# ubc-vision/quadraturefields

Measured on AMD Instinct MI355X. Metric: rays/sec at 800x800 Lego (mesh-quadrature render: ray/mesh intersection + hash-grid/MLP field + compositing), higher is better.
Workload: dtype f32; 1 GPU; Lego 800x800 (configs[1]), 1xMI355X per frame, fp32 hash-grid + tiny-MLP HIP kernels; rays_per_frame=640000, max_hits=25, triangles=983040, log2_hashmap_size=19, up_sample=1, bvh_fallback_frames=0, overflow_repaired_frames=8, reorigin_rule_redone_frames=0, camera_mismatch_frames=0, frames_in_flight=1

## Files before the change

quadraturefields_amd/build.py:

```python
import os
import subprocess
import sys
from concurrent.futures import ThreadPoolExecutor

PKG_DIR = os.path.dirname(os.path.abspath(__file__))
ROOT = os.path.dirname(PKG_DIR)
CSRC = os.path.join(PKG_DIR, "csrc")
OBJ_DIR = os.path.join(CSRC, "_obj")
LIB_PATH = os.path.join(PKG_DIR, "libqf_hip.so")
ARCH = "gfx950"

SOURCES = [
    ("field_eval.hip", []),
    ("field_eval_bf16.hip", []),
    ("grid_extract.hip", []),
    ("grid_backward.hip", []),
    ("mlp_train.hip", []),
    ("field_train.hip", []),
    ("scan.hip", []),
    ("composite.hip", []),
    ("distortion.hip", []),
    ("optim.hip", []),
    ("frame_metrics.hip", []),
    ("bvh_traverse.hip", ["-ffp-contract=off"]),
    ("raster.hip", ["-ffp-contract=off"]),
    ("sample_pack.hip", ["-ffp-contract=off"]),
    ("texture.hip", ["-ffp-contract=off"]),
    ("bake.hip", ["-ffp-contract=off"]),
    ("grid_march.hip", ["-ffp-contract=off"]),
    ("volumetric.hip", ["-ffp-contract=off"]),
    ("texel_fill.hip", ["-ffp-contract=off"]),
    ("marching_cubes.hip", ["-ffp-contract=off"]),
    ("vertex_clustering.hip", ["-ffp-contract=off"]),
    ("uv_atlas.hip", ["-ffp-contract=off"]),
    ("bvh_build_device.hip", ["-ffp-contract=off"]),
    ("bvh_build.cpp", ["-x", "hip"]),
    ("misc.cpp", ["-x", "hip"]),
    ("frame.cpp", ["-x", "hip"]),
]
COMMON = os.environ.get("QF_EXTRA_HIPCC_FLAGS", "").split() + ["-O3", "-std=c++17", "-fPIC", f"--offload-arch={ARCH}", "-I" + os.path.join(ROOT, "include"),
          "-I" + CSRC, "-Wall", "-Wno-unused-function"]


def _hipcc() -> str:
    for cand in (os.environ.get("HIPCC"), "/opt/rocm/bin/hipcc", "hipcc"):
        if cand and (os.path.isabs(cand) and os.path.exists(cand) or not os.path.isabs(cand)):
            return cand
    raise RuntimeError("hipcc not found")


def _deps(src: str):
    deps = [os.path.join(CSRC, src), os.path.join(ROOT, "include", "qf_hip.h"), os.path.abspath(__file__)]
    deps += [os.path.join(CSRC, f) for f in os.listdir(CSRC) if f.endswith(".h")]
    return deps


def _stale(target: str, deps) -> bool:
    if not os.path.exists(target):
        return True
    t = os.path.getmtime(target)
    return any(os.path.getmtime(d) > t for d in deps)


def _obj(src: str) -> str:
    return os.path.join(OBJ_DIR, os.path.splitext(src)[0] + ".o")


def _compile(item):
    src, extra = item
    obj = _obj(src)
    if not _stale(obj, _deps(src)):
        return obj, False
    cmd = [_hipcc()] + COMMON + extra + ["-c", os.path.join(CSRC, src), "-o", obj]
    proc = subprocess.run(cmd, capture_output=True, text=True)
    if proc.returncode != 0:
        raise RuntimeError("hipcc failed for %s:\n%s\n%s" % (src, " ".join(cmd), proc.stderr))
    if proc.stderr.strip():
        sys.stderr.write(proc.stderr)
    return obj, True


def build(force: bool = False, verbose: bool = False) -> str:
    os.makedirs(OBJ_DIR, exist_ok=True)
    keep = set() if force else {_obj(src) for src, _ in SOURCES}
    for f in os.listdir(OBJ_DIR):
        if os.path.join(OBJ_DIR, f) not in keep:
            os.remove(os.path.join(OBJ_DIR, f))
    with ThreadPoolExecutor(max_workers=4) as pool:
        results = list(pool.map(_compile, SOURCES))
    objs = [o for o, _ in results]
    if any(changed for _, changed in results) or _stale(LIB_PATH, objs):
        cmd = [_hipcc(), "-shared", "-fPIC", f"--offload-arch={ARCH}", "-o", LIB_PATH] + objs
        proc = subprocess.run(cmd, capture_output=True, text=True)
        if proc.returncode != 0:
            raise RuntimeError("link failed:\n%s\n%s" % (" ".join(cmd), proc.stderr))
        if verbose:
            print("linked", LIB_PATH)
    return LIB_PATH


if __name__ == "__main__":
    print(build(force="--force" in sys.argv, verbose=True))
```

quadraturefields_amd/csrc/raster.hip:

```cpp
#include <type_traits>

#include "exact_common.h"

#pragma clang fp contract(off)

namespace {

struct RasterCam {
    float r00, r01, r02, r10, r11, r12, r20, r21, r22;
    float cx, cy, cz;
    float fx, fy, px0, py0;
    int w, h;
};

constexpr float kRasterGuard = 0.25f;

struct SlabArgs {
    float t_lo, t_hi;
    int stop_at;
    uint64_t *keys;
    const float4 *ray_rec;
};

struct TriSetup {
    int x0, x1, y0, y1;
    bool use_edges;
    float ea[3], eb[3], ec[3];
};

__device__ __forceinline__ bool tri_setup(const float4 a, const float4 b, const float4 c, const RasterCam &cam, TriSetup &s)
{
    float minx = INFINITY, maxx = -INFINITY, miny = INFINITY, maxy = -INFINITY;
    int behind = 0;
    const float4 vs[3] = {a, b, c};
    float sxs[3], sys[3];
#pragma unroll
    for (int k = 0; k < 3; ++k) {
        const float dx = vs[k].x - cam.cx, dy = vs[k].y - cam.cy, dz = vs[k].z - cam.cz;
        const float xc = cam.r00 * dx + cam.r10 * dy + cam.r20 * dz;
        const float yc = cam.r01 * dx + cam.r11 * dy + cam.r21 * dz;
        const float zc = cam.r02 * dx + cam.r12 * dy + cam.r22 * dz;
        const float zv = -zc;
        if (!(zv > 1e-6f)) { ++behind; sxs[k] = sys[k] = 0.0f; continue; }
        const float sx = cam.fx * (xc / zv) + cam.px0;
        const float sy = -cam.fy * (yc / zv) + cam.py0;
        sxs[k] = sx; sys[k] = sy;
        minx = fminf(minx, sx); maxx = fmaxf(maxx, sx);
        miny = fminf(miny, sy); maxy = fmaxf(maxy, sy);
    }
    if (behind == 3) return false;
    s.use_edges = false;
    if (behind > 0) {
        s.x0 = 0; s.y0 = 0; s.x1 = cam.w - 1; s.y1 = cam.h - 1;
    } else {
        s.x0 = (int)fmaxf(floorf(minx - kRasterGuard), 0.0f);
        s.y0 = (int)fmaxf(floorf(miny - kRasterGuard), 0.0f);
        s.x1 = (int)fminf(ceilf(maxx + kRasterGuard), (float)(cam.w - 1));
        s.y1 = (int)fminf(ceilf(maxy + kRasterGuard), (float)(cam.h - 1));
        if (!(maxx + kRasterGuard >= 0.0f) || !(maxy + kRasterGuard >= 0.0f) ||
            !(minx - kRasterGuard <= (float)(cam.w - 1)) || !(miny - kRasterGuard <= (float)(cam.h - 1)))
            return false;
        const float area2 = (sxs[1] - sxs[0]) * (sys[2] - sys[0]) - (sys[1] - sys[0]) * (sxs[2] - sxs[0]);
        if (fabsf(area2) > 1e-2f) {
            s.use_edges = true;
            const float sgn = area2 > 0.0f ? 1.0f : -1.0f;
#pragma unroll
            for (int k = 0; k < 3; ++k) {
                const int k1 = (k + 1) % 3;
                const float ex = sxs[k1] - sxs[k], ey = sys[k1] - sys[k];
                s.ea[k] = -sgn * ey;
                s.eb[k] = sgn * ex;
                s.ec[k] = -(s.ea[k] * sxs[k] + s.eb[k] * sys[k]) + (kRasterGuard + 0.05f) * (fabsf(ex) + fabsf(ey)) + 1e-3f;
            }
        }
    }
    return true;
}

constexpr int kBinStage = 256;
constexpr int kBinIdBits = 26;
struct BinStage { int n; int tile[kBinStage]; uint2 rec[kBinStage]; };
struct TileBins {
    int32_t *cursor;
    uint2 *bins;
    int cap;
    BinStage *stage;
};

__device__ __forceinline__ void bin_records(const TileBins &tb, int tile, uint2 rec)
{
    const int lane = (int)__lane_id();
    for (;;) {
        const int t0 = __builtin_amdgcn_readfirstlane(tile);
        const unsigned long long m = __ballot(tile == t0);
        if (tile == t0) {
            const int rank = __popcll(m & ((1ull << lane) - 1ull));
            int base = 0;
            if (rank == 0) base = atomicAdd(&tb.cursor[t0], __popcll(m));
            base = __shfl(base, __ffsll((long long)m) - 1, 64);
            if (base + rank < tb.cap) tb.bins[(int64_t)t0 * tb.cap + base + rank] = rec;
            break;
        }
    }
}

template <int kRasterLanes, bool kWide, bool kSlab = false, bool kBins = false>
__device__ __forceinline__ void raster_triangle(const float4 *__restrict__ tris, int64_t tri_i, int sub, const RasterCam &cam,
                                                const float *__restrict__ rays_o, const float *__restrict__ rays_d,
                                                int max_hits, int32_t *__restrict__ hit_tri, float *__restrict__ hit_t,
                                                int32_t *__restrict__ hit_count, int32_t *__restrict__ overflow,
                                                const bool cam_origin, const SlabArgs slab = SlabArgs(),
                                                const TileBins bins = TileBins())
{
    const float4 a = tris[tri_i * 3 + 0], b = tris[tri_i * 3 + 1], c = tris[tri_i * 3 + 2];
    const int id = __float_as_int(a.w);
    TriSetup ts;
    if (!tri_setup(a, b, c, cam, ts)) return;
    const int x0 = ts.x0, x1 = ts.x1, y0 = ts.y0, y1 = ts.y1;
    const bool use_edges = ts.use_edges;
    const float *ea = ts.ea, *eb = ts.eb, *ec = ts.ec;
    const int bw = x1 - x0 + 1;
    const int total = bw * (y1 - y0 + 1);
    int px = x0 + sub % bw, py = y0 + sub / bw;
    for (int q = sub; q < total; q += kRasterLanes) {
        const int cx_ = px, cy_ = py;
        px += kRasterLanes;
        while (px > x1) { px -= bw; ++py; }
        if (use_edges) {
            const float fx_ = (float)cx_, fy_ = (float)cy_;
            if (ea[0] * fx_ + eb[0] * fy_ + ec[0] < 0.0f || ea[1] * fx_ + eb[1] * fy_ + ec[1] < 0.0f ||
                ea[2] * fx_ + eb[2] * fy_ + ec[2] < 0.0f)
                continue;
        }
        const int64_t ray = (int64_t)cy_ * cam.w + cx_;
        float dx, dy, dz;
        if (kSlab && slab.ray_rec) {
            const float4 rr = slab.ray_rec[ray];
            if (__float_as_int(rr.w) >= slab.stop_at) continue;
            dx = rr.x; dy = rr.y; dz = rr.z;
        } else {
            dx = rays_d[ray * 3]; dy = rays_d[ray * 3 + 1]; dz = rays_d[ray * 3 + 2];
        }
        float ox = cam.cx, oy = cam.cy, oz = cam.cz;
        if (!cam_origin) { ox = rays_o[ray * 3]; oy = rays_o[ray * 3 + 1]; oz = rays_o[ray * 3 + 2]; }
        asm volatile("" : "+v"(ox), "+v"(oy), "+v"(oz), "+v"(dx), "+v"(dy), "+v"(dz));
        float t;
        if (!mt_hit(a, b, c, ox, oy, oz, dx, dy, dz, &t)) continue;
        if (kSlab) {
            if (!(t >= slab.t_lo && t < slab.t_hi)) continue;
            const int slot = atomicAdd(&hit_count[ray], 1);
            if (slot < max_hits) slab.keys[(int64_t)slot * ((int64_t)cam.w * cam.h) + ray] = hit_key(t, id);
            else atomicAdd(overflow, 1);
            continue;
        }
        if (kBins) {
            const int tile = (cy_ >> 3) * ((cam.w + 7) >> 3) + (cx_ >> 3);
            const uint2 rec = make_uint2(__float_as_uint(t), ((uint32_t)id << 6) | (uint32_t)((cy_ & 7) * 8 + (cx_ & 7)));
            const int at = atomicAdd(&bins.stage->n, 1);
            if (at < kBinStage) { bins.stage->tile[at] = tile; bins.stage->rec[at] = rec; }
            else bin_records(bins, tile, rec);
            continue;
        }
        const int slot = atomicAdd(&hit_count[ray], 1);
        if (slot < max_hits) {
            const int64_t at = kWide ? (int64_t)slot * ((int64_t)cam.w * cam.h) + ray : ray * max_hits + slot;
            hit_t[at] = t;
            if (hit_tri) hit_tri[at] = id;
        } else {
            atomicAdd(overflow, 1);
        }
    }
}

template <int kRasterLanes, bool kWide>
__global__ __launch_bounds__(256) void raster_kernel(const float4 *__restrict__ tris, int64_t n_tri, RasterCam cam,
                                                     const float *__restrict__ rays_o, const float *__restrict__ rays_d,
                                                     int max_hits, int32_t *__restrict__ hit_tri, float *__restrict__ hit_t,
                                                     int32_t *__restrict__ hit_count, int32_t *__restrict__ overflow,
                                                     const int32_t *__restrict__ ray_flag)
{
    const int64_t gid = (int64_t)blockIdx.x * blockDim.x + threadIdx.x;
    const int64_t tri_i = gid / kRasterLanes;
    const int sub = (int)(gid % kRasterLanes);
    if (tri_i >= n_tri) return;
    if (ray_flag && *ray_flag) return;
    const bool cam_origin = ray_flag != nullptr;
    raster_triangle<kRasterLanes, kWide>(tris, tri_i, sub, cam, rays_o, rays_d, max_hits, hit_tri, hit_t, hit_count, overflow,
                                         cam_origin);
}

template <int kRasterLanes>
__global__ __launch_bounds__(256) void raster_bins_kernel(const float4 *__restrict__ tris, int64_t n_tri, RasterCam cam,
                                                          const float *__restrict__ rays_o, const float *__restrict__ rays_d,
                                                          int max_hits, int32_t *__restrict__ tile_cursor,
                                                          uint2 *__restrict__ bin_records_out,
                                                          const int32_t *__restrict__ ray_flag)
{
    __shared__ BinStage s_stage[4];
    const int64_t gid = (int64_t)blockIdx.x * blockDim.x + threadIdx.x;
    const int64_t tri_i = gid / kRasterLanes;
    const int sub = (int)(gid % kRasterLanes);
    if (ray_flag && *ray_flag) return;
    const bool cam_origin = ray_flag != nullptr;
    const int lane = (int)(threadIdx.x & 63);
    TileBins tb;
    tb.cursor = tile_cursor;
    tb.bins = bin_records_out;
    tb.cap = 64 * max_hits;
    tb.stage = &s_stage[threadIdx.x >> 6];
    if (lane == 0) tb.stage->n = 0;
    __builtin_amdgcn_fence(__ATOMIC_ACQ_REL, "workgroup");
    __builtin_amdgcn_wave_barrier();
    if (tri_i < n_tri)
        raster_triangle<kRasterLanes, false, false, true>(tris, tri_i, sub, cam, rays_o, rays_d, max_hits, nullptr, nullptr,
                                                          nullptr, nullptr, cam_origin, SlabArgs(), tb);
    __builtin_amdgcn_fence(__ATOMIC_ACQ_REL, "workgroup");
    __builtin_amdgcn_wave_barrier();
    const int n = tb.stage->n < kBinStage ? tb.stage->n : kBinStage;
    for (int i = lane; i < n; i += 64) bin_records(tb, tb.stage->tile[i], tb.stage->rec[i]);
}

__global__ __launch_bounds__(64) void tile_count_kernel(const int32_t *__restrict__ tile_cursor, const uint2 *__restrict__ bins,
                                                        int max_hits, int w, int h, int tiles_x,
                                                        int32_t *__restrict__ hit_count, int32_t *__restrict__ overflow,
                                                        uint64_t *__restrict__ tile_mask)
{
    __shared__ int s_cnt[64];
    const int tile = blockIdx.x, lane = threadIdx.x;
    const int cap = 64 * max_hits;
    const int cursor = tile_cursor[tile];
    const int n = cursor < cap ? cursor : cap;
    const int px = (tile % tiles_x) * 8 + (lane & 7), py = (tile / tiles_x) * 8 + (lane >> 3);
    const bool inside = px < w && py < h;
    int c = 0;
    if (n > 0) {
        s_cnt[lane] = 0;
        __syncthreads();
        const uint2 *run = bins + (int64_t)tile * cap;
        for (int i = lane; i < n; i += 64) atomicAdd(&s_cnt[run[i].y & 63u], 1);
        __syncthreads();
        c = s_cnt[lane];
    }
    int over = c > max_hits ? c - max_hits : 0;
    if (cursor > cap) {
        c = c > max_hits ? c : max_hits + 1;
        over = lane == 0 ? cursor - cap : 0;
    }
    if (inside) hit_count[(int64_t)py * w + px] = c;
    const unsigned long long mask = __ballot(inside && c > max_hits);
    if (mask) {
#pragma unroll
        for (int off = 32; off > 0; off >>= 1) over += __shfl_xor(over, off, 64);
        if (lane == 0) atomicAdd(overflow, over);
    }
    if (lane == 0) tile_mask[tile] = mask;
}

constexpr float kRayPixelTol = 0.02f;
constexpr float kRayUnitTol = 1e-4f;

__device__ __forceinline__ void camera_rays_check(const uint32_t *__restrict__ o_bits, const float *__restrict__ rays_d,
                                                  int64_t n_rays, const RasterCam &cam, int32_t *__restrict__ flag,
                                                  int64_t first, int64_t stride)
{
    const uint32_t c0 = __float_as_uint(cam.cx), c1 = __float_as_uint(cam.cy), c2 = __float_as_uint(cam.cz);
    bool bad = false;
    for (int64_t r = first; r < n_rays; r += stride) {
        const uint32_t o0 = o_bits[r * 3], o1 = o_bits[r * 3 + 1], o2 = o_bits[r * 3 + 2];
        const float dx = rays_d[r * 3], dy = rays_d[r * 3 + 1], dz = rays_d[r * 3 + 2];
        bad = bad || o0 != c0 || o1 != c1 || o2 != c2;
        const float xc = cam.r00 * dx + cam.r10 * dy + cam.r20 * dz;
        const float yc = cam.r01 * dx + cam.r11 * dy + cam.r21 * dz;
        const float zv = -(cam.r02 * dx + cam.r12 * dy + cam.r22 * dz);
        const float sx = cam.fx * (xc / zv) + cam.px0, sy = -cam.fy * (yc / zv) + cam.py0;
        const float px = (float)(int)(r % cam.w), py = (float)(int)(r / cam.w);
        bad = bad || !(zv > 0.0f) || !(fabsf(sx - px) <= kRayPixelTol) || !(fabsf(sy - py) <= kRayPixelTol) ||
              !(fabsf(dx * dx + dy * dy + dz * dz - 1.0f) <= kRayUnitTol);
    }
    if (bad) *flag = 1;
}

__global__ void camera_rays_check_kernel(const uint32_t *__restrict__ o_bits, const float *__restrict__ rays_d, int64_t n_rays,
                                         RasterCam cam, int32_t *__restrict__ flag)
{
    camera_rays_check(o_bits, rays_d, n_rays, cam, flag, (int64_t)blockIdx.x * blockDim.x + threadIdx.x,
                      (int64_t)gridDim.x * blockDim.x);
}

constexpr int kCullChunk = 64;

__global__ __launch_bounds__(256) void chunk_boxes_kernel(const float4 *__restrict__ tris, int64_t n_tri, int n_chunks,
                                                          float4 *__restrict__ boxes)
{
    const int chunk = (int)(((int64_t)blockIdx.x * blockDim.x + threadIdx.x) >> 6), lane = threadIdx.x & 63;
    if (chunk >= n_chunks) return;
    const int64_t t = (int64_t)chunk * kCullChunk + lane;
    float lo[3] = {INFINITY, INFINITY, INFINITY}, hi[3] = {-INFINITY, -INFINITY, -INFINITY};
    if (t < n_tri) {
#pragma unroll
        for (int k = 0; k < 3; ++k) {
            const float4 v = tris[t * 3 + k];
            lo[0] = fminf(lo[0], v.x); lo[1] = fminf(lo[1], v.y); lo[2] = fminf(lo[2], v.z);
            hi[0] = fmaxf(hi[0], v.x); hi[1] = fmaxf(hi[1], v.y); hi[2] = fmaxf(hi[2], v.z);
        }
    }
#pragma unroll
    for (int off = 32; off > 0; off >>= 1) {
#pragma unroll
        for (int k = 0; k < 3; ++k) {
            lo[k] = fminf(lo[k], __shfl_xor(lo[k], off, 64));
            hi[k] = fmaxf(hi[k], __shfl_xor(hi[k], off, 64));
        }
    }
    if (lane == 0) {
        boxes[chunk * 2 + 0] = make_float4(lo[0], lo[1], lo[2], 0.0f);
        boxes[chunk * 2 + 1] = make_float4(hi[0], hi[1], hi[2], 0.0f);
    }
}

__global__ void cull_chunks_kernel(const float4 *__restrict__ boxes, int n_chunks, RasterCam cam, int32_t *__restrict__ visible,
                                   int32_t *__restrict__ counters, int parity, const uint32_t *__restrict__ o_bits,
                                   const float *__restrict__ rays_d, int64_t n_rays, int32_t *__restrict__ ray_flag)
{
    const int chunk = blockIdx.x * blockDim.x + threadIdx.x;
    if (chunk == 0) counters[parity ^ 1] = 0;
    if (ray_flag) camera_rays_check(o_bits, rays_d, n_rays, cam, ray_flag, chunk, (int64_t)gridDim.x * blockDim.x);
    if (chunk >= n_chunks) return;
    const float4 lo = boxes[chunk * 2], hi = boxes[chunk * 2 + 1];
    if (!(lo.x <= hi.x)) return;
    float minx = INFINITY, maxx = -INFINITY, miny = INFINITY, maxy = -INFINITY;
    bool keep = false;
#pragma unroll
    for (int k = 0; k < 8; ++k) {
        const float dx = ((k & 1) ? hi.x : lo.x) - cam.cx, dy = ((k & 2) ? hi.y : lo.y) - cam.cy, dz = ((k & 4) ? hi.z : lo.z) - cam.cz;
        const float xc = cam.r00 * dx + cam.r10 * dy + cam.r20 * dz;
        const float yc = cam.r01 * dx + cam.r11 * dy + cam.r21 * dz;
        const float zc = cam.r02 * dx + cam.r12 * dy + cam.r22 * dz;
        const float zv = -zc;
        if (!(zv > 1e-4f)) { keep = true; continue; }
        const float sx = cam.fx * (xc / zv) + cam.px0, sy = -cam.fy * (yc / zv) + cam.py0;
        minx = fminf(minx, sx); maxx = fmaxf(maxx, sx);
        miny = fminf(miny, sy); maxy = fmaxf(maxy, sy);
    }
    const float g = kRasterGuard + 1.0f;
    if (!keep)
        keep = (maxx + g >= 0.0f) && (maxy + g >= 0.0f) && (minx - g <= (float)(cam.w - 1)) && (miny - g <= (float)(cam.h - 1));
    if (keep) visible[atomicAdd(&counters[parity], 1)] = chunk;
}

template <int kRasterLanes, bool kWide>
__global__ __launch_bounds__(256) void raster_culled_kernel(const float4 *__restrict__ tris, int64_t n_tri, RasterCam cam,
                                                            const float *__restrict__ rays_o, const float *__restrict__ rays_d,
                                                            int max_hits, int32_t *__restrict__ hit_tri, float *__restrict__ hit_t,
                                                            int32_t *__restrict__ hit_count, int32_t *__restrict__ overflow,
                                                            const int32_t *__restrict__ visible, const int32_t *__restrict__ n_visible,
                                                            const int32_t *__restrict__ ray_flag)
{
    if (ray_flag && *ray_flag) return;
    const bool cam_origin = ray_flag != nullptr;
    constexpr int kTrisPerBlock = 256 / kRasterLanes;
    constexpr int kBlocksPerChunk = kCullChunk / kTrisPerBlock;
    const int n_items = *n_visible * kBlocksPerChunk;
    const int sub = threadIdx.x % kRasterLanes;
    for (int item = blockIdx.x; item < n_items; item += gridDim.x) {
        const int chunk = visible[item / kBlocksPerChunk];
        const int64_t tri_i = (int64_t)chunk * kCullChunk + (item % kBlocksPerChunk) * kTrisPerBlock + threadIdx.x / kRasterLanes;
        if (tri_i < n_tri)
            raster_triangle<kRasterLanes, kWide>(tris, tri_i, sub, cam, rays_o, rays_d, max_hits, hit_tri, hit_t, hit_count, overflow,
                                                 cam_origin);
    }
}

constexpr int kMaxSlabs = 16;

struct SlabCtl {
    uint32_t dist_min_bits, dist_max_bits;
    int32_t n_visible;
    int32_t slab_count[kMaxSlabs];
};

__device__ __forceinline__ void slab_range(const SlabCtl *ctl, int n_slabs, float *lo, float *width)
{
    const float dmin = __uint_as_float(ctl->dist_min_bits) * 0.999f, dmax = __uint_as_float(ctl->dist_max_bits) * 1.001f;
    *lo = dmin;
    *width = fmaxf(dmax - dmin, 1e-12f) / (float)n_slabs;
}

__device__ __forceinline__ void slab_edges(const SlabCtl *ctl, int n_slabs, int j, float *t_lo, float *t_hi)
{
#pragma clang fp contract(off)
    float lo, w;
    slab_range(ctl, n_slabs, &lo, &w);
    *t_lo = j == 0 ? -INFINITY : lo + (float)j * w;
    *t_hi = j == n_slabs - 1 ? INFINITY : lo + (float)(j + 1) * w;
}

__global__ void slab_init_kernel(SlabCtl *ctl)
{
    ctl->dist_min_bits = 0x7f800000u;
    ctl->dist_max_bits = 0u;
    ctl->n_visible = 0;
    for (int j = 0; j < kMaxSlabs; ++j) ctl->slab_count[j] = 0;
}

__global__ void slab_cull_kernel(const float4 *__restrict__ boxes, int n_chunks, RasterCam cam, int32_t *__restrict__ visible,
                                 float2 *__restrict__ range, SlabCtl *ctl)
{
    const int chunk = blockIdx.x * blockDim.x + threadIdx.x;
    if (chunk >= n_chunks) return;
    const float4 lo = boxes[chunk * 2], hi = boxes[chunk * 2 + 1];
    if (!(lo.x <= hi.x)) return;
    float minx = INFINITY, maxx = -INFINITY, miny = INFINITY, maxy = -INFINITY;
    bool keep = false;
#pragma unroll
    for (int k = 0; k < 8; ++k) {
        const float dx = ((k & 1) ? hi.x : lo.x) - cam.cx, dy = ((k & 2) ? hi.y : lo.y) - cam.cy, dz = ((k & 4) ? hi.z : lo.z) - cam.cz;
        const float xc = cam.r00 * dx + cam.r10 * dy + cam.r20 * dz;
        const float yc = cam.r01 * dx + cam.r11 * dy + cam.r21 * dz;
        const float zc = cam.r02 * dx + cam.r12 * dy + cam.r22 * dz;
        const float zv = -zc;
        if (!(zv > 1e-4f)) { keep = true; continue; }
        const float sx = cam.fx * (xc / zv) + cam.px0, sy = -cam.fy * (yc / zv) + cam.py0;
        minx = fminf(minx, sx); maxx = fmaxf(maxx, sx);
        miny = fminf(miny, sy); maxy = fmaxf(maxy, sy);
    }
    const float g = kRasterGuard + 1.0f;
    if (!keep)
        keep = (maxx + g >= 0.0f) && (maxy + g >= 0.0f) && (minx - g <= (float)(cam.w - 1)) && (miny - g <= (float)(cam.h - 1));
    if (!keep) return;
    const float nx = fmaxf(fmaxf(lo.x - cam.cx, cam.cx - hi.x), 0.0f), ny = fmaxf(fmaxf(lo.y - cam.cy, cam.cy - hi.y), 0.0f);
    const float nz = fmaxf(fmaxf(lo.z - cam.cz, cam.cz - hi.z), 0.0f);
    const float fx = fmaxf(fabsf(lo.x - cam.cx), fabsf(hi.x - cam.cx)), fy = fmaxf(fabsf(lo.y - cam.cy), fabsf(hi.y - cam.cy));
    const float fz = fmaxf(fabsf(lo.z - cam.cz), fabsf(hi.z - cam.cz));
    const float dmin = sqrtf(nx * nx + ny * ny + nz * nz) * 0.9999f, dmax = sqrtf(fx * fx + fy * fy + fz * fz) * 1.0001f + 1e-30f;
    visible[atomicAdd(&ctl->n_visible, 1)] = chunk;
    range[chunk] = make_float2(dmin, dmax);
    atomicMin(&ctl->dist_min_bits, __float_as_uint(dmin));
    atomicMax(&ctl->dist_max_bits, __float_as_uint(dmax));
}

__global__ __launch_bounds__(256) void slab_assign_kernel(const int32_t *__restrict__ visible, const float2 *__restrict__ range,
                                                          SlabCtl *ctl, int n_slabs, int n_chunks, int32_t *__restrict__ lists)
{
    __shared__ int s_cnt[kMaxSlabs], s_base[kMaxSlabs];
    if (threadIdx.x < kMaxSlabs) s_cnt[threadIdx.x] = 0;
    __syncthreads();
    const int e = blockIdx.x * blockDim.x + threadIdx.x;
    int chunk = -1, j0 = 0, j1 = -1;
    if (e < ctl->n_visible) {
        chunk = visible[e];
        const float2 r = range[chunk];
        const float dlo = r.x * 0.999f, dhi = r.y * 1.001f;
        j0 = n_slabs;
        for (int j = 0; j < n_slabs; ++j) {
            float t_lo, t_hi;
            slab_edges(ctl, n_slabs, j, &t_lo, &t_hi);
            if (t_hi > dlo && t_lo <= dhi) { j0 = j < j0 ? j : j0; j1 = j; }
        }
        for (int j = j0; j <= j1; ++j) atomicAdd(&s_cnt[j], 1);
    }
    __syncthreads();
    if (threadIdx.x < n_slabs) s_base[threadIdx.x] = s_cnt[threadIdx.x] ? atomicAdd(&ctl->slab_count[threadIdx.x], s_cnt[threadIdx.x]) : 0;
    __syncthreads();
    for (int j = j0; j <= j1; ++j) lists[(int64_t)j * n_chunks + atomicAdd(&s_base[j], 1)] = chunk;
}

__global__ void slab_ray_records_kernel(const float *__restrict__ rays_d, const int32_t *__restrict__ hit_count, int64_t n,
                                        float4 *__restrict__ rec)
{
    for (int64_t i = (int64_t)blockIdx.x * blockDim.x + threadIdx.x; i < n; i += (int64_t)gridDim.x * blockDim.x)
        rec[i] = make_float4(rays_d[i * 3], rays_d[i * 3 + 1], rays_d[i * 3 + 2], __int_as_float(hit_count[i]));
}

template <int kRasterLanes>
// ... 545 lines not shown
```

Measured before the change: 409.0 million rays/s.

## Split triangle setup across a lane quad with DPP and specialize the pixel loop on ray origin

Each lane in a quad now projects one triangle vertex, and the projections and edge equations are exchanged with DPP quad permutes. Before, every lane projected all three vertices redundantly. The pixel walk moves into a helper header that drops the modulo and divide, and the loop is specialized at compile time on whether the ray origin is the camera. SLP vectorization is disabled for the raster file. Risks are extra DPP moves, quad-alignment assumptions that are only checked by a static_assert, and changed code generation from the new compiler flag.

```diff
diff --git a/quadraturefields_amd/build.py b/quadraturefields_amd/build.py
--- a/quadraturefields_amd/build.py
+++ b/quadraturefields_amd/build.py
@@ -23,7 +23,7 @@
     ("optim.hip", []),
     ("frame_metrics.hip", []),
     ("bvh_traverse.hip", ["-ffp-contract=off"]),
-    ("raster.hip", ["-ffp-contract=off"]),
+    ("raster.hip", ["-ffp-contract=off", "-fno-slp-vectorize"]),
     ("sample_pack.hip", ["-ffp-contract=off"]),
     ("texture.hip", ["-ffp-contract=off"]),
     ("bake.hip", ["-ffp-contract=off"]),
diff --git a/quadraturefields_amd/csrc/raster.hip b/quadraturefields_amd/csrc/raster.hip
--- a/quadraturefields_amd/csrc/raster.hip
+++ b/quadraturefields_amd/csrc/raster.hip
@@ -1,6 +1,7 @@
 #include <type_traits>
 
 #include "exact_common.h"
+#include "raster_walk.h"
 
 #pragma clang fp contract(off)
 
@@ -28,52 +29,65 @@
     float ea[3], eb[3], ec[3];
 };
 
-__device__ __forceinline__ bool tri_setup(const float4 a, const float4 b, const float4 c, const RasterCam &cam, TriSetup &s)
-{
+constexpr int kQuadLane0 = 0x00, kQuadLane1 = 0x55, kQuadLane2 = 0xAA;
+constexpr int kQuadNext3 = 0xC9;
+template <int kCtrl>
+__device__ __forceinline__ float quad_read(float v)
+{
+    return __int_as_float(__builtin_amdgcn_update_dpp(0, __float_as_int(v), kCtrl, 0xf, 0xf, true));
+}
+
+__device__ __forceinline__ bool tri_setup(const float4 a, const float4 b, const float4 c, const RasterCam &cam, int sub, TriSetup &s)
+{
+    const int q = sub & 3;
+    const float vx = q == 0 ? a.x : (q == 1 ? b.x : c.x);
+    const float vy = q == 0 ? a.y : (q == 1 ? b.y : c.y);
+    const float vz = q == 0 ? a.z : (q == 1 ? b.z : c.z);
+    const float dx = vx - cam.cx, dy = vy - cam.cy, dz = vz - cam.cz;
+    const float xc = cam.r00 * dx + cam.r10 * dy + cam.r20 * dz;
+    const float yc = cam.r01 * dx + cam.r11 * dy + cam.r21 * dz;
+    const float zc = cam.r02 * dx + cam.r12 * dy + cam.r22 * dz;
+    const float zv = -zc;
+    const bool front = zv > 1e-6f;
+    const float sx = front ? cam.fx * (xc / zv) + cam.px0 : 0.0f;
+    const float sy = front ? -cam.fy * (yc / zv) + cam.py0 : 0.0f;
+    const float fr = front ? 1.0f : 0.0f;
+    const float sxs[3] = {quad_read<kQuadLane0>(sx), quad_read<kQuadLane1>(sx), quad_read<kQuadLane2>(sx)};
+    const float sys[3] = {quad_read<kQuadLane0>(sy), quad_read<kQuadLane1>(sy), quad_read<kQuadLane2>(sy)};
+    const int behind = 3 - (int)(quad_read<kQuadLane0>(fr) + quad_read<kQuadLane1>(fr) + quad_read<kQuadLane2>(fr));
+    if (behind == 3) return false;
     float minx = INFINITY, maxx = -INFINITY, miny = INFINITY, maxy = -INFINITY;
-    int behind = 0;
-    const float4 vs[3] = {a, b, c};
-    float sxs[3], sys[3];
 #pragma unroll
     for (int k = 0; k < 3; ++k) {
-        const float dx = vs[k].x - cam.cx, dy = vs[k].y - cam.cy, dz = vs[k].z - cam.cz;
-        const float xc = cam.r00 * dx + cam.r10 * dy + cam.r20 * dz;
-        const float yc = cam.r01 * dx + cam.r11 * dy + cam.r21 * dz;
-        const float zc = cam.r02 * dx + cam.r12 * dy + cam.r22 * dz;
-        const float zv = -zc;
-        if (!(zv > 1e-6f)) { ++behind; sxs[k] = sys[k] = 0.0f; continue; }
-        const float sx = cam.fx * (xc / zv) + cam.px0;
-        const float sy = -cam.fy * (yc / zv) + cam.py0;
-        sxs[k] = sx; sys[k] = sy;
-        minx = fminf(minx, sx); maxx = fmaxf(maxx, sx);
-        miny = fminf(miny, sy); maxy = fmaxf(maxy, sy);
-    }
-    if (behind == 3) return false;
-    s.use_edges = false;
-    if (behind > 0) {
-        s.x0 = 0; s.y0 = 0; s.x1 = cam.w - 1; s.y1 = cam.h - 1;
-    } else {
-        s.x0 = (int)fmaxf(floorf(minx - kRasterGuard), 0.0f);
-        s.y0 = (int)fmaxf(floorf(miny - kRasterGuard), 0.0f);
-        s.x1 = (int)fminf(ceilf(maxx + kRasterGuard), (float)(cam.w - 1));
-        s.y1 = (int)fminf(ceilf(maxy + kRasterGuard), (float)(cam.h - 1));
+        minx = fminf(minx, sxs[k]); maxx = fmaxf(maxx, sxs[k]);
+        miny = fminf(miny, sys[k]); maxy = fmaxf(maxy, sys[k]);
+    }
+    int x0 = 0, y0 = 0, x1 = cam.w - 1, y1 = cam.h - 1;
+    bool use_edges = false;
+    float ea0 = 0.0f, ea1 = 0.0f, ea2 = 0.0f, eb0 = 0.0f, eb1 = 0.0f, eb2 = 0.0f, ec0 = 0.0f, ec1 = 0.0f, ec2 = 0.0f;
+    if (behind == 0) {
+        x0 = (int)fmaxf(floorf(minx - kRasterGuard), 0.0f);
+        y0 = (int)fmaxf(floorf(miny - kRasterGuard), 0.0f);
+        x1 = (int)fminf(ceilf(maxx + kRasterGuard), (float)(cam.w - 1));
+        y1 = (int)fminf(ceilf(maxy + kRasterGuard), (float)(cam.h - 1));
         if (!(maxx + kRasterGuard >= 0.0f) || !(maxy + kRasterGuard >= 0.0f) ||
             !(minx - kRasterGuard <= (float)(cam.w - 1)) || !(miny - kRasterGuard <= (float)(cam.h - 1)))
             return false;
+        if (x1 < x0 || y1 < y0) return false;
         const float area2 = (sxs[1] - sxs[0]) * (sys[2] - sys[0]) - (sys[1] - sys[0]) * (sxs[2] - sxs[0]);
         if (fabsf(area2) > 1e-2f) {
-            s.use_edges = true;
+            use_edges = true;
             const float sgn = area2 > 0.0f ? 1.0f : -1.0f;
-#pragma unroll
-            for (int k = 0; k < 3; ++k) {
-                const int k1 = (k + 1) % 3;
-                const float ex = sxs[k1] - sxs[k], ey = sys[k1] - sys[k];
-                s.ea[k] = -sgn * ey;
-                s.eb[k] = sgn * ex;
-                s.ec[k] = -(s.ea[k] * sxs[k] + s.eb[k] * sys[k]) + (kRasterGuard + 0.05f) * (fabsf(ex) + fabsf(ey)) + 1e-3f;
-            }
-        }
-    }
+            const float ex = quad_read<kQuadNext3>(sx) - sx, ey = quad_read<kQuadNext3>(sy) - sy;
+            const float ea = -sgn * ey;
+            const float eb = sgn * ex;
+            const float ec = -(ea * sx + eb * sy) + (kRasterGuard + 0.05f) * (fabsf(ex) + fabsf(ey)) + 1e-3f;
+            ea0 = quad_read<kQuadLane0>(ea); ea1 = quad_read<kQuadLane1>(ea); ea2 = quad_read<kQuadLane2>(ea);
+            eb0 = quad_read<kQuadLane0>(eb); eb1 = quad_read<kQuadLane1>(eb); eb2 = quad_read<kQuadLane2>(eb);
+            ec0 = quad_read<kQuadLane0>(ec); ec1 = quad_read<kQuadLane1>(ec); ec2 = quad_read<kQuadLane2>(ec);
+        }
+    }
+    s = TriSetup{x0, x1, y0, y1, use_edges, {ea0, ea1, ea2}, {eb0, eb1, eb2}, {ec0, ec1, ec2}};
     return true;
 }
 
@@ -114,62 +128,64 @@
 {
     const float4 a = tris[tri_i * 3 + 0], b = tris[tri_i * 3 + 1], c = tris[tri_i * 3 + 2];
     const int id = __float_as_int(a.w);
+    static_assert(kRasterLanes % 4 == 0 && 256 % kRasterLanes == 0, "a quad of lanes never spans two triangles (tri_setup)");
     TriSetup ts;
-    if (!tri_setup(a, b, c, cam, ts)) return;
+    if (!tri_setup(a, b, c, cam, sub, ts)) return;
     const int x0 = ts.x0, x1 = ts.x1, y0 = ts.y0, y1 = ts.y1;
     const bool use_edges = ts.use_edges;
-    const float *ea = ts.ea, *eb = ts.eb, *ec = ts.ec;
-    const int bw = x1 - x0 + 1;
-    const int total = bw * (y1 - y0 + 1);
-    int px = x0 + sub % bw, py = y0 + sub / bw;
-    for (int q = sub; q < total; q += kRasterLanes) {
-        const int cx_ = px, cy_ = py;
-        px += kRasterLanes;
-        while (px > x1) { px -= bw; ++py; }
-        if (use_edges) {
-            const float fx_ = (float)cx_, fy_ = (float)cy_;
-            if (ea[0] * fx_ + eb[0] * fy_ + ec[0] < 0.0f || ea[1] * fx_ + eb[1] * fy_ + ec[1] < 0.0f ||
-                ea[2] * fx_ + eb[2] * fy_ + ec[2] < 0.0f)
+    const float ea[3] = {ts.ea[0], ts.ea[1], ts.ea[2]}, eb[3] = {ts.eb[0], ts.eb[1], ts.eb[2]}, ec[3] = {ts.ec[0], ts.ec[1], ts.ec[2]};
+    auto pixels = [=](auto origin_is_cam) {
+        constexpr bool kCamOrigin = decltype(origin_is_cam)::value;
+        QfRasterWalk walk = qf_raster_walk_begin(x0, y0, x1, sub);
+        for (; !qf_raster_walk_done(walk, y1); qf_raster_walk_step(walk, x0, x1, kRasterLanes)) {
+            if (use_edges) {
+                const float fx_ = (float)walk.px, fy_ = (float)walk.py;
+                if (ea[0] * fx_ + eb[0] * fy_ + ec[0] < 0.0f || ea[1] * fx_ + eb[1] * fy_ + ec[1] < 0.0f ||
+                    ea[2] * fx_ + eb[2] * fy_ + ec[2] < 0.0f)
+                    continue;
+            }
+            const int cx_ = walk.px, cy_ = walk.py;
+            const int64_t ray = (int64_t)cy_ * cam.w + cx_;
+            float dx, dy, dz;
+            if (kSlab && slab.ray_rec) {
+                const float4 rr = slab.ray_rec[ray];
+                if (__float_as_int(rr.w) >= slab.stop_at) continue;
+                dx = rr.x; dy = rr.y; dz = rr.z;
+            } else {
+                dx = rays_d[ray * 3]; dy = rays_d[ray * 3 + 1]; dz = rays_d[ray * 3 + 2];
+            }
+            float ox = cam.cx, oy = cam.cy, oz = cam.cz;
+            if (!kCamOrigin) { ox = rays_o[ray * 3]; oy = rays_o[ray * 3 + 1]; oz = rays_o[ray * 3 + 2]; }
+            asm volatile("" : "+v"(ox), "+v"(oy), "+v"(oz), "+v"(dx), "+v"(dy), "+v"(dz));
+            float t;
+            if (!mt_hit(a, b, c, ox, oy, oz, dx, dy, dz, &t)) continue;
+            if (kSlab) {
+                if (!(t >= slab.t_lo && t < slab.t_hi)) continue;
+                const int slot = atomicAdd(&hit_count[ray], 1);
+                if (slot < max_hits) slab.keys[(int64_t)slot * ((int64_t)cam.w * cam.h) + ray] = hit_key(t, id);
+                else atomicAdd(overflow, 1);
                 continue;
-        }
-        const int64_t ray = (int64_t)cy_ * cam.w + cx_;
-        float dx, dy, dz;
-        if (kSlab && slab.ray_rec) {
-            const float4 rr = slab.ray_rec[ray];
-            if (__float_as_int(rr.w) >= slab.stop_at) continue;
-            dx = rr.x; dy = rr.y; dz = rr.z;
-        } else {
-            dx = rays_d[ray * 3]; dy = rays_d[ray * 3 + 1]; dz = rays_d[ray * 3 + 2];
-        }
-        float ox = cam.cx, oy = cam.cy, oz = cam.cz;
-        if (!cam_origin) { ox = rays_o[ray * 3]; oy = rays_o[ray * 3 + 1]; oz = rays_o[ray * 3 + 2]; }
-        asm volatile("" : "+v"(ox), "+v"(oy), "+v"(oz), "+v"(dx), "+v"(dy), "+v"(dz));
-        float t;
-        if (!mt_hit(a, b, c, ox, oy, oz, dx, dy, dz, &t)) continue;
-        if (kSlab) {
-            if (!(t >= slab.t_lo && t < slab.t_hi)) continue;
+            }
+            if (kBins) {
+                const int tile = (cy_ >> 3) * ((cam.w + 7) >> 3) + (cx_ >> 3);
+                const uint2 rec = make_uint2(__float_as_uint(t), ((uint32_t)id << 6) | (uint32_t)((cy_ & 7) * 8 + (cx_ & 7)));
+                const int at = atomicAdd(&bins.stage->n, 1);
+                if (at < kBinStage) { bins.stage->tile[at] = tile; bins.stage->rec[at] = rec; }
+                else bin_records(bins, tile, rec);
+                continue;
+            }
             const int slot = atomicAdd(&hit_count[ray], 1);
-            if (slot < max_hits) slab.keys[(int64_t)slot * ((int64_t)cam.w * cam.h) + ray] = hit_key(t, id);
-            else atomicAdd(overflow, 1);
-            continue;
-        }
-        if (kBins) {
-            const int tile = (cy_ >> 3) * ((cam.w + 7) >> 3) + (cx_ >> 3);
-            const uint2 rec = make_uint2(__float_as_uint(t), ((uint32_t)id << 6) | (uint32_t)((cy_ & 7) * 8 + (cx_ & 7)));
-            const int at = atomicAdd(&bins.stage->n, 1);
-            if (at < kBinStage) { bins.stage->tile[at] = tile; bins.stage->rec[at] = rec; }
-            else bin_records(bins, tile, rec);
-            continue;
-        }
-        const int slot = atomicAdd(&hit_count[ray], 1);
-        if (slot < max_hits) {
-            const int64_t at = kWide ? (int64_t)slot * ((int64_t)cam.w * cam.h) + ray : ray * max_hits + slot;
-            hit_t[at] = t;
-            if (hit_tri) hit_tri[at] = id;
-        } else {
-            atomicAdd(overflow, 1);
-        }
-    }
+            if (slot < max_hits) {
+                const int64_t at = kWide ? (int64_t)slot * ((int64_t)cam.w * cam.h) + ray : ray * max_hits + slot;
+                hit_t[at] = t;
+                if (hit_tri) hit_tri[at] = id;
+            } else {
+                atomicAdd(overflow, 1);
+            }
+        }
+    };
+    if (cam_origin) pixels(std::true_type());
+    else pixels(std::false_type());
 }
 
 template <int kRasterLanes, bool kWide>
diff --git a/quadraturefields_amd/csrc/raster_walk.h b/quadraturefields_amd/csrc/raster_walk.h
--- /dev/null
+++ b/quadraturefields_amd/csrc/raster_walk.h
@@ -0,0 +1,36 @@
+#pragma once
+
+#ifdef __HIPCC__
+#define QF_WALK_FN __host__ __device__ __forceinline__
+#else
+#define QF_WALK_FN inline
+#endif
+
+struct QfRasterWalk {
+    int px, py;
+};
+
+QF_WALK_FN void qf_raster_walk_wrap(QfRasterWalk &w, int x1, int bw)
+{
+    while (w.px > x1) {
+        w.px -= bw;
+        ++w.py;
+    }
+}
+
+QF_WALK_FN QfRasterWalk qf_raster_walk_begin(int x0, int y0, int x1, int sub)
+{
+    QfRasterWalk w;
+    w.px = x0 + sub;
+    w.py = y0;
+    qf_raster_walk_wrap(w, x1, x1 - x0 + 1);
+    return w;
+}
+
+QF_WALK_FN bool qf_raster_walk_done(const QfRasterWalk &w, int y1) { return w.py > y1; }
+
+QF_WALK_FN void qf_raster_walk_step(QfRasterWalk &w, int x0, int x1, int lanes)
+{
+    w.px += lanes;
+    qf_raster_walk_wrap(w, x1, x1 - x0 + 1);
+}
```

After: 412.3 million rays/s (median of 6 runs). About the same (+0.8%).
